# mynameisfiber/baton

Hardware: NVIDIA H100
Metric: federated local samples/sec (whole box), ResNet-18 FedAvg, synthetic non-IID 32x32 shards (higher is better)
Workload: dtype bf16

## Files before the change

### baton_b200/csrc/bindings.cpp

```cpp
#include <ATen/cuda/CUDAContext.h>
#include <c10/cuda/CUDAGuard.h>
#include <torch/extension.h>

#include <optional>
#include <vector>

#include "launch.h"

namespace {

inline cudaStream_t cur_stream() { return at::cuda::getCurrentCUDAStream().stream(); }
inline void check(int rc, const char* what) {
  TORCH_CHECK(rc == 0, "baton_b200::", what, " failed with code ", rc,
              rc > 0 ? std::string(" (") + cudaGetErrorString(static_cast<cudaError_t>(rc)) + ")" : std::string());
}
inline const void* cptr(const at::Tensor& t) { return t.data_ptr(); }
inline void* ptr(at::Tensor& t) { return t.data_ptr(); }
template <class T>
inline T* opt_ptr(const std::optional<at::Tensor>& t) {
  return (t.has_value() && t->defined()) ? reinterpret_cast<T*>(t->data_ptr()) : nullptr;
}
#define CHECK_CUDA(x) TORCH_CHECK((x).is_cuda(), #x " must be a CUDA tensor")

inline const float* prox_anchor(const std::optional<at::Tensor>& anchor, int64_t numel, const at::Tensor& hyper) {
// ... 289 lines not shown
  const int64_t nout = out.numel() / rows;
  TORCH_CHECK(w.numel() == (dgrad ? c * 9 * nout : nout * 9 * c), "conv_smallmap: w must be [Cout, 9*Cin]");
  TORCH_CHECK(dgrad ? !col_stats.has_value()
                    : (!col_stats.has_value() || (col_stats->scalar_type() == at::kFloat && col_stats->numel() >= 2 * nout)),
              "conv_smallmap: col_stats is a [2 Cout] fp32 buffer of the forward");
  const c10::cuda::CUDAGuard guard(src.device());
  const int rc = b200_conv_smallmap(cptr(src), cptr(w), ptr(out), static_cast<int>(src.size(0)),
                                    static_cast<int>(src.size(1)), static_cast<int>(src.size(2)), static_cast<int>(c),
                                    static_cast<int>(nout), static_cast<int>(stride), dgrad ? 1 : 0, static_cast<int>(mc),
                                    static_cast<int>(bn), opt_ptr<float>(col_stats), cur_stream());
  if (rc == -2) return false;
  check(rc, "conv_smallmap");
  return true;
}
bool conv_igemm_dgrad_s2(const at::Tensor& dy, const at::Tensor& w, at::Tensor dx, int64_t kh, int64_t kw,
                         const std::vector<int64_t>& ntaps, const std::vector<int64_t>& taps, int64_t force_bn) {
  CHECK_CUDA(dy); CHECK_CUDA(w); CHECK_CUDA(dx);
  TORCH_CHECK(dy.scalar_type() == at::kBFloat16 && w.scalar_type() == at::kBFloat16 && dx.scalar_type() == at::kBFloat16 &&
              dy.dim() == 4 && dx.dim() == 4 && dy.is_contiguous() && w.is_contiguous() && dx.is_contiguous());
  TORCH_CHECK(ntaps.size() == 4 && taps.size() == 16, "conv_igemm_dgrad_s2: 4 classes x 4 taps");
  int nt[4], tw[16];
  for (int i = 0; i < 4; ++i) nt[i] = static_cast<int>(ntaps[i]);
  for (int i = 0; i < 16; ++i) tw[i] = static_cast<int>(taps[i]);
  const c10::cuda::CUDAGuard guard(dy.device());
  const int rc = b200_conv_igemm_dgrad_s2(cptr(dy), cptr(w), ptr(dx), static_cast<int>(dx.size(0)),
                                          static_cast<int>(dx.size(1)), static_cast<int>(dx.size(2)),
                                          static_cast<int>(dx.size(3)), static_cast<int>(dy.size(3)), static_cast<int>(kh),
                                          static_cast<int>(kw), static_cast<int>(dy.size(1)), static_cast<int>(dy.size(2)),
                                          nt, tw, static_cast<int>(force_bn), cur_stream());
  if (rc == -2) return false;
  check(rc, "conv_igemm_dgrad_s2");
  return true;
}
bool conv_igemm_wgrad(const at::Tensor& dy, const at::Tensor& x, at::Tensor dw, int64_t cout, int64_t kh, int64_t kw,
                      int64_t stride, int64_t pad, int64_t ho, int64_t wo, int64_t split_k, int64_t force_bn,
                      const std::optional<at::Tensor>& sgd_theta, const std::optional<at::Tensor>& sgd_theta_bf16,
                      const std::optional<at::Tensor>& sgd_mom, const std::optional<at::Tensor>& sgd_hyper,
                      bool sgd_nesterov, const std::optional<at::Tensor>& sgd_anchor,
                      const std::optional<at::Tensor>& sgd_corr, const std::optional<at::Tensor>& sgd_v) {
  CHECK_CUDA(dy); CHECK_CUDA(x); CHECK_CUDA(dw);
  TORCH_CHECK(x.scalar_type() == at::kBFloat16 && dy.scalar_type() == at::kBFloat16 && dw.scalar_type() == at::kFloat &&
              x.dim() == 4 && x.is_contiguous() && dy.is_contiguous());
  const c10::cuda::CUDAGuard guard(x.device());
  const std::optional<B200SgdEpilogue> sgd =
      sgd_epilogue(sgd_theta, sgd_theta_bf16, sgd_mom, sgd_hyper, sgd_nesterov, sgd_anchor, sgd_corr, sgd_v);
  const int rc = b200_conv_igemm_wgrad(cptr(dy), cptr(x), dw.data_ptr<float>(), static_cast<int>(x.size(0)),
                                       static_cast<int>(x.size(1)), static_cast<int>(x.size(2)), static_cast<int>(x.size(3)),
                                       static_cast<int>(cout), static_cast<int>(kh), static_cast<int>(kw),
                                       static_cast<int>(stride), static_cast<int>(pad), static_cast<int>(ho),
                                       static_cast<int>(wo), static_cast<int>(split_k), static_cast<int>(force_bn),
                                       sgd ? &*sgd : nullptr, cur_stream());
  if (rc == -2 || rc == B200_SGD_EPILOGUE_DECLINED) return false;
  check(rc, "conv_igemm_wgrad");
  return true;
}

void gemm_fp8(const at::Tensor& a, const at::Tensor& b, at::Tensor d, const std::optional<at::Tensor>& bias,
              const std::optional<at::Tensor>& sfa, const std::optional<at::Tensor>& sfb, int64_t M, int64_t N, int64_t K,
              int64_t lda, int64_t ldb, int64_t ldd, int64_t act, int64_t split_k, bool accumulate, double alpha) {
  CHECK_CUDA(a); CHECK_CUDA(b); CHECK_CUDA(d);
  TORCH_CHECK(a.element_size() == 1 && b.element_size() == 1, "gemm_fp8 operands must be 1-byte (e4m3)");
  const c10::cuda::CUDAGuard guard(a.device());
  check(b200_gemm_fp8(cptr(a), cptr(b), ptr(d), opt_ptr<const float>(bias), opt_ptr<const void>(sfa),
                      opt_ptr<const void>(sfb), M, N, K, lda, ldb, ldd, d.scalar_type() == at::kFloat, act, split_k,
                      accumulate, static_cast<float>(alpha), cur_stream()),
        "gemm_fp8");
}
void quant_mx_rows(const at::Tensor& x, at::Tensor q, at::Tensor sf, int64_t R, int64_t C, int64_t ld_in, int64_t Cp) {
  CHECK_CUDA(x);
  const c10::cuda::CUDAGuard guard(x.device());
  check(b200_quant_mx_rows(x.data_ptr(), q.data_ptr(), sf.data_ptr(), R, C, ld_in, Cp, cur_stream()), "quant_mx_rows");
}
void quant_mx_cols(const at::Tensor& x, at::Tensor q, at::Tensor sf, int64_t R, int64_t C, int64_t ld_in, int64_t Rp) {
  CHECK_CUDA(x);
  const c10::cuda::CUDAGuard guard(x.device());
  check(b200_quant_mx_cols(x.data_ptr(), q.data_ptr(), sf.data_ptr(), R, C, ld_in, Rp, cur_stream()), "quant_mx_cols");
}

void fused_sgd(at::Tensor w, at::Tensor g, const std::optional<at::Tensor>& mom, const std::optional<at::Tensor>& wb,
               const at::Tensor& hyper, bool zero_grad, bool nesterov, const std::optional<at::Tensor>& wire_slot,
               const std::optional<at::Tensor>& pack_global, const std::optional<at::Tensor>& pack_scale, int64_t n_pack,
               bool wire_fp32, const std::optional<at::Tensor>& prox_anchor_, const std::optional<at::Tensor>& corr,
               const std::optional<at::Tensor>& adam_v, bool clip) {
  CHECK_CUDA(w);
  TORCH_CHECK(w.scalar_type() == at::kFloat && g.scalar_type() == at::kFloat && hyper.scalar_type() == at::kFloat);
  TORCH_CHECK(w.is_contiguous() && g.is_contiguous() && w.numel() == g.numel());
  const c10::cuda::CUDAGuard guard(w.device());
  const float* anchor = prox_anchor(prox_anchor_, w.numel(), hyper);
  const float* c = scaf_corr(corr, w.numel(), anchor);
  float* v = adam_v_ptr(adam_v, w.numel(), opt_ptr<float>(mom), hyper, anchor, c);
  check_clip_hyper(clip, hyper, v != nullptr);
  check(b200_fused_sgd(w.data_ptr<float>(), g.data_ptr<float>(), opt_ptr<float>(mom), opt_ptr<void>(wb), w.numel(),
                       hyper.data_ptr<float>(), zero_grad, nesterov,
                       reinterpret_cast<const unsigned long long*>(opt_ptr<const int64_t>(wire_slot)),
                       opt_ptr<const float>(pack_global), opt_ptr<const float>(pack_scale), n_pack, wire_fp32, anchor,
                       c, v, clip ? 1 : 0, cur_stream()),
        "fused_sgd");
}

void fused_sgd_segments(at::Tensor w, at::Tensor g, const std::optional<at::Tensor>& mom,
                        const std::optional<at::Tensor>& wb, const at::Tensor& segments, const at::Tensor& hyper,
                        bool nesterov, const std::optional<at::Tensor>& prox_anchor_,
                        const std::optional<at::Tensor>& corr, const std::optional<at::Tensor>& adam_v, bool clip) {
  CHECK_CUDA(w); CHECK_CUDA(segments);
  TORCH_CHECK(w.scalar_type() == at::kFloat && g.scalar_type() == at::kFloat && hyper.scalar_type() == at::kFloat);
  TORCH_CHECK(segments.scalar_type() == at::kLong && segments.dim() == 2 && segments.size(1) == 3 &&
// ... 1161 lines not shown
                            d.scalar_type() == at::kFloat, static_cast<int>(act), static_cast<float>(alpha), &l,
                            cur_stream()),
        "gemm_bf16_lora");
}

void lora_down(const at::Tensor& x, int64_t ldx, const at::Tensor& w, int64_t w_ts, int64_t wsj, int64_t wsk,
               at::Tensor u, int64_t ldu, int64_t M, int64_t T, int64_t rs, int64_t kt, const std::vector<int64_t>& xoff) {
  check_bf16(x, "lora_down x"); check_bf16(w, "lora_down w"); check_bf16(u, "lora_down u");
  TORCH_CHECK(static_cast<int64_t>(xoff.size()) == T, "lora_down: one x offset per slice");
  const c10::cuda::CUDAGuard guard(x.device());
  std::vector<long long> xo(xoff.begin(), xoff.end());
  check(b200_lora_down(cptr(x), ldx, cptr(w), w_ts, wsj, wsk, ptr(u), ldu, M, T, rs, kt, xo.data(), cur_stream()),
        "lora_down");
}

void lora_grad(const at::Tensor& l, int64_t ldl, const at::Tensor& q, int64_t ldq, at::Tensor out, int64_t osa,
               int64_t osb, int64_t out_ts, int64_t M, int64_t NA, int64_t NB, int64_t T, const std::vector<int64_t>& lo,
               const std::vector<int64_t>& qo, double s, at::Tensor work) {
  check_bf16(l, "lora_grad l"); check_bf16(q, "lora_grad q");
  CHECK_CUDA(out); CHECK_CUDA(work);
  TORCH_CHECK(out.scalar_type() == at::kFloat && work.scalar_type() == at::kFloat, "lora_grad: fp32 out and work");
  TORCH_CHECK(static_cast<int64_t>(lo.size()) == T && static_cast<int64_t>(qo.size()) == T, "lora_grad: offsets per slice");
  const int64_t splits = (M + B200_LORA_SPLIT_ROWS - 1) / B200_LORA_SPLIT_ROWS;
  TORCH_CHECK(work.numel() >= T * splits * NA * NB, "lora_grad: work holds T * splits * NA * NB floats");
  const c10::cuda::CUDAGuard guard(l.device());
  std::vector<long long> lo_(lo.begin(), lo.end()), qo_(qo.begin(), qo.end());
  check(b200_lora_grad(cptr(l), ldl, cptr(q), ldq, out.data_ptr<float>(), osa, osb, out_ts, M, NA, NB, T, lo_.data(),
                       qo_.data(), static_cast<float>(s), work.data_ptr<float>(), cur_stream()),
        "lora_grad");
}

}

PYBIND11_MODULE(TORCH_EXTENSION_NAME, m) {
  m.doc() = "baton_b200 sm_90a kernels";
  m.attr("MAX_RANKS") = B200_MAX_RANKS;
  m.def("gemm", &gemm);
  m.def("gemm_lora", &gemm_lora);
  m.def("lora_down", &lora_down);
  m.def("lora_grad", &lora_grad);
  m.attr("LORA_MAX_R") = B200_LORA_MAX_R;
  m.attr("LORA_SPLIT_ROWS") = B200_LORA_SPLIT_ROWS;
  m.def("trace_set", &trace_set);
  m.def("attention_fwd", &attention_fwd);
  m.def("attention_bwd", &attention_bwd);
  m.def("attention_short_fwd", &attention_short_fwd);
  m.def("attention_short_bwd", &attention_short_bwd);
  m.def("bn_bwd_cluster", &bn_bwd_cluster);
  m.def("gn_fwd", &gn_fwd);
  m.def("gn_bwd", &gn_bwd);
  m.def("im2col_tma_probe", &im2col_tma_probe);
  m.def("conv_igemm_fwd", &conv_igemm_fwd);
  m.def("conv_igemm_wgrad", &conv_igemm_wgrad);
  m.def("conv_igemm_dgrad", &conv_igemm_dgrad);
  m.def("conv_igemm_dgrad_s2", &conv_igemm_dgrad_s2);
  m.def("conv_halo", &conv_halo);
  m.def("conv_smallmap", &conv_smallmap);
  m.def("gemm_batched", &gemm_batched);
  m.def("gemm_fp8", &gemm_fp8);
  m.def("quant_mx_rows", &quant_mx_rows);
  m.def("quant_mx_cols", &quant_mx_cols);
  m.def("fused_sgd", &fused_sgd);
  m.def("fused_sgd_segments", &fused_sgd_segments);
  m.def("grad_norm_clip", &grad_norm_clip);
  m.attr("GRAD_NORM_WORK_WORDS") = B200_GRAD_NORM_WORK_WORDS;
  m.def("weighted_sum", &weighted_sum);
  m.def("fold_client", &fold_client);
  m.def("scaffold_corr", &scaffold_corr);
  m.def("scaffold_dc", &scaffold_dc);
  m.def("cast", &cast);
  m.def("gather_rows", &gather_rows);
  m.def("gather_augment", &gather_augment);
  m.def("gather_mix", &gather_mix);
  m.def("colsum", &colsum);
  m.def("add_bf16", &add_bf16);
  m.def("relu_bwd", &relu_bwd);
  m.def("gelu", &gelu);
  m.def("gelu_bwd", &gelu_bwd);
  m.def("gelu_erf", &gelu_erf);
  m.def("gelu_erf_bwd", &gelu_erf_bwd);
  m.def("vit_tokens_fwd", &vit_tokens_fwd);
  m.def("vit_tokens_bwd", &vit_tokens_bwd);
  m.def("pad_rows", &pad_rows);
  m.def("embedding_bwd", &embedding_bwd);
  m.def("fedavg_allreduce", &fedavg_allreduce);
  m.def("fedavg_allreduce_robust", &fedavg_allreduce_robust);
  m.def("fedavg_allreduce_krum", &fedavg_allreduce_krum);
  m.attr("KRUM_MAX_CTAS") = B200_KRUM_MAX_CTAS;
  m.attr("KRUM_PAIRS") = B200_KRUM_PAIRS;
  m.attr("KRUM_REPORT") = B200_KRUM_REPORT;
  m.def("fedavg_allreduce_topk", &fedavg_allreduce_topk);
  m.def("fedavg_allreduce_local", &fedavg_allreduce_local);
  m.def("fedavg_allreduce_secagg", &fedavg_allreduce_secagg);
  m.def("secagg_encode", &secagg_encode);
  m.def("topk_pack", &topk_pack);
  m.def("topk_fold", &topk_fold);
  m.def("nonzero_pack", &nonzero_pack);
  m.def("topk_work_words", [](int64_t n) { return static_cast<int64_t>(B200_TOPK_WORK_WORDS(n)); });
  m.def("pack_client", &pack_client);
  m.attr("MAX_ROBUST_CLIENTS") = B200_MAX_ROBUST_CLIENTS;
  m.attr("DP_WORK_WORDS") = B200_DP_WORK_WORDS;
  m.def("dp_clip_factor", &dp_clip_factor);
  m.def("fold_client_scaled", &fold_client_scaled);
  m.def("im2col", &im2col);
  m.def("col2im", &col2im);
  m.def("maxpool", &maxpool);
// ... 31 lines not shown
```

### baton_b200/csrc/gemm_wgmma.cu

```cuda
#define B200_TU_TAG 1
#include "ptx.cuh"
#include "epilogue.cuh"
#include "launch.h"
#include "pdl.cuh"
#include "sgd.cuh"

namespace b200 {

constexpr int BM = 128;
constexpr int BK = 64;
constexpr int WG_K = 16;
constexpr int GEMM_THREADS = 384;
constexpr int CONSUMER_WARPS = 8;
constexpr int CONSUMER_THREADS = 32 * CONSUMER_WARPS;
constexpr int MAX_STAGES = 8;
constexpr int S2_MAX_TAPS = 4;

struct GemmParams {
  int M, N, K;
  void* D;
  long long ldd;
  const float* bias;
  int out_fp32;
  int act;
// ... 1555 lines not shown
  p.ldb = static_cast<long long>(KH) * KW * Cin;
  p.flag_bias_off = -1; p.flag_epoch_ptr = nullptr;
  p.batched = 0; p.batch_inner = 1; p.batch_count = 1; p.d_outer = 0; p.d_inner = 0;
  p.conv_ho = Ho; p.conv_wo = Wo; p.conv_stride = 2; p.conv_pad = 0; p.conv_kw = KW; p.conv_cin = Cout;
  p.conv_taps = KH * KW; p.conv_ncol = Cin; p.conv_h = H; p.conv_w = W;
  dim3 grid((Cin + bn - 1) / bn, static_cast<unsigned>(4 * tiles_m), 1);
  if (bn == 128) return launch_fixed<128, 6, 4>(ta, tb, p, grid, stream);
  return launch_fixed<64, 8, 4>(ta, tb, p, grid, stream);
}

extern "C" int b200_conv_igemm_wgrad(const void* dy, const void* x, float* dw, int N, int H, int W, int Cin, int Cout,
                                     int KH, int KW, int stride, int pad, int Ho, int Wo, int split_k, int force_bn,
                                     const B200SgdEpilogue* sgd, cudaStream_t stream) {
  using namespace b200;
  const long long Mp = static_cast<long long>(N) * Ho * Wo;
  const int Kc = KH * KW * Cin;
  if (Mp <= 0 || Cout <= 0) return 0;
  if (Cin % 64 != 0 || Cout % 8 != 0 || Mp > (1ll << 30) || (reinterpret_cast<uintptr_t>(x) & 15) ||
      (reinterpret_cast<uintptr_t>(dy) & 15) || (reinterpret_cast<uintptr_t>(dw) & 15))
    return -2;
  const int bn = clamp_bn(force_bn > 0 ? force_bn : (Kc > 64 ? 128 : 64));
  CUtensorMap ta, tb;
  int rc = make_map(&ta, dy, Mp, Cout, Cout, 64, BK);
  if (rc) return rc;
  rc = b200_encode_map_im2col_bf16(&tb, x, N, H, W, Cin, KH, KW, stride, pad, 64, 64);
  if (rc) return rc;
  const int k_tiles = static_cast<int>((Mp + BK - 1) / BK);
  if (split_k < 1) split_k = 1;
  if (split_k > k_tiles) split_k = k_tiles;
  const int per = (k_tiles + split_k - 1) / split_k;
  split_k = (k_tiles + per - 1) / per;
  if (sgd != nullptr && split_k != 1) return B200_SGD_EPILOGUE_DECLINED;
  GemmParams p;
  if (sgd != nullptr) set_sgd_epilogue(p, *sgd);
  p.M = Cout; p.N = Kc; p.K = static_cast<int>(Mp); p.D = dw; p.ldd = Kc; p.bias = nullptr; p.out_fp32 = 1; p.act = 0;
  p.a_mn = 1; p.b_mn = 1; p.k_tiles_per_split = per; p.cluster_k = 1; p.atomic_out = 1;
  p.col_stats = nullptr;
  p.tile_flags = nullptr; p.flag_epoch = 0; p.alpha = 1.0f; p.flag_elem_off = 0; p.flag_tile_elems = 0; p.ldb = Kc;
  p.flag_bias_off = -1; p.flag_epoch_ptr = nullptr;
  p.batched = 0; p.batch_inner = 1; p.batch_count = 1; p.d_outer = 0; p.d_inner = 0;
  p.stages = 4;
  p.conv_ho = Ho; p.conv_wo = Wo; p.conv_stride = stride; p.conv_pad = pad; p.conv_kw = KW; p.conv_cin = Cin;
  p.conv_taps = KH * KW; p.conv_ncol = Cin;
  dim3 grid((Kc + bn - 1) / bn, (Cout + BM - 1) / BM, split_k);
  if (sgd != nullptr) {
    if (bn == 128) return launch_fixed_sgd<128, 6, 2>(ta, tb, p, grid, stream);
    return launch_fixed_sgd<64, 8, 2>(ta, tb, p, grid, stream);
  }
  if (bn == 128) return launch_fixed<128, 6, 2>(ta, tb, p, grid, stream);
  return launch_fixed<64, 8, 2>(ta, tb, p, grid, stream);
}

B200_TRACE_REGISTER(gemm_wgmma)
```

### baton_b200/csrc/launch.h

```cpp
#pragma once
#include <cuda_runtime.h>
#include <stdint.h>

#define B200_MAX_RANKS 16

extern "C" {

struct B200SgdEpilogue {
  float* theta;
  void* theta_bf16;
  float* mom;
  const float* hyper;
  int nesterov;
  const float* anchor;
  const float* corr;
  float* v;
};
#define B200_SGD_EPILOGUE_DECLINED (-6)

struct B200AffineEpilogue {
  const float* scale;
  const float* shift;
  const void* residual;
  long long ldr;
// ... 3 lines not shown

#define B200_LORA_MAX_R 192
struct B200LoraEpilogue {
  const void* u;
  long long ldu;
  const void* f;
  long long fs_n, fs_j;
  int R, rs, ds;
  int slot[3];
  float s;
};
int b200_gemm_bf16_lora(const void* a, const void* b, void* d, const float* bias, int M, int N, int K, long long lda,
                        long long ldb, long long ldd, int a_mn, int b_mn, int out_fp32, int act, float alpha,
                        const B200LoraEpilogue* lora, cudaStream_t stream);
int b200_lora_down(const void* x, long long ldx, const void* w, long long w_ts, long long wsj, long long wsk, void* u,
                   long long ldu, int M, int T, int rs, int kt, const long long* xoff, cudaStream_t stream);
#define B200_LORA_SPLIT_ROWS 256
int b200_lora_grad(const void* l, long long ldl, const void* q, long long ldq, float* out, long long osa, long long osb,
                   long long out_ts, int M, int NA, int NB, int T, const long long* lo, const long long* qo, float s,
                   float* work, cudaStream_t stream);

int b200_gemm_bf16(const void* a, const void* b, void* d, const float* bias, int M, int N, int K, long long lda,
                   long long ldb, long long ldd, int a_mn, int b_mn, int out_fp32, int act, int split_k, int accumulate,
                   float alpha, const uint32_t* tile_flags, uint32_t flag_epoch, long long flag_elem_off, int flag_tile_elems,
                   long long flag_bias_off, int force_bn, float* col_stats, const uint32_t* flag_epoch_ptr,
                   const B200SgdEpilogue* sgd, const B200AffineEpilogue* affine, cudaStream_t stream);
int b200_gemm_bf16_batched(const void* a, const void* b, void* d, int M, int N, int K, long long lda, long long ldb,
                           long long ldd, int a_mn, int b_mn, int out_fp32, int act, float alpha, int n_outer,
                           int n_inner, long long a_outer, long long a_inner, long long b_outer, long long b_inner,
                           long long d_outer, long long d_inner, int accumulate, cudaStream_t stream);
int b200_attention_fwd(const void* qkv, void* out, void* probs, int B, int S, int H, int dh, float scale,
                       cudaStream_t stream);
int b200_attention_bwd(const void* qkv, const void* dout, const void* probs, void* dqkv, int B, int S, int H, int dh,
                       float scale, cudaStream_t stream);
struct B200Dropout;
int b200_attention_drop_fwd(const void* qkv, void* out, void* probs, int B, int S, int H, int dh, float scale,
                            const B200Dropout* drop, cudaStream_t stream);
int b200_attention_drop_bwd(const void* qkv, const void* dout, const void* probs, void* dqkv, int B, int S, int H, int dh,
                            float scale, const B200Dropout* drop, cudaStream_t stream);
int b200_attention_short_fwd(const void* qkv, void* out, void* probs, int B, int S, int H, int dh, float scale,
                             cudaStream_t stream);
int b200_attention_short_bwd(const void* qkv, const void* dout, const void* probs, void* dqkv, int B, int S, int H, int dh,
                             float scale, cudaStream_t stream);
int b200_conv_igemm_fwd(const void* x, const void* w, void* y, int N, int H, int W, int Cin, int Cout, int KH, int KW,
                        int stride, int pad, int Ho, int Wo, int cluster_k, int force_bn, float* col_stats,
                        const B200AffineEpilogue* affine, cudaStream_t stream);
int b200_conv_igemm_dgrad(const void* dy, const void* w, void* dx, int N, int H, int W, int Cin, int Cout, int KH, int KW,
                          int pad, int Ho, int Wo, int cluster_k, int force_bn, cudaStream_t stream);
int b200_conv_igemm_dgrad_s2(const void* dy, const void* w, void* dx, int N, int H, int W, int Cin, int Cout, int KH,
                             int KW, int Ho, int Wo, const int* ntaps, const int* taps, int force_bn, cudaStream_t stream);
int b200_conv_igemm_wgrad(const void* dy, const void* x, float* dw, int N, int H, int W, int Cin, int Cout, int KH, int KW,
                          int stride, int pad, int Ho, int Wo, int split_k, int force_bn, const B200SgdEpilogue* sgd,
                          cudaStream_t stream);
int b200_conv_halo(const void* src, const void* w, void* out, int N, int H, int W, int C, int Nout, int stride,
                   int dgrad, int mc, float* col_stats, cudaStream_t stream);
int b200_conv_smallmap(const void* src, const void* w, void* out, int N, int H, int W, int C, int Nout, int stride,
                       int dgrad, int mc, int bn, float* col_stats, cudaStream_t stream);
int b200_im2col_tma_probe(const void* x, void* col, int N, int H, int W, int C, int KH, int KW, int stride, int pad,
                          int Ho, int Wo, cudaStream_t stream);
int b200_gemm_fp8(const void* a, const void* b, void* d, const float* bias, const void* sfa, const void* sfb, int M, int N,
                  int K, long long lda, long long ldb, long long ldd, int out_fp32, int act, int split_k, int accumulate,
                  float alpha, cudaStream_t stream);
int b200_quant_mx_rows(const void* x, void* q, void* sf, long long R, int C, long long ld_in, int Cp, cudaStream_t stream);
int b200_quant_mx_cols(const void* x, void* q, void* sf, long long R, int C, long long ld_in, long long Rp,
                       cudaStream_t stream);
int b200_gemm_simt(const void* a, const void* b, void* d, const float* bias, int M, int N, int K, long long lda,
                   long long ldb, long long ldd, int a_mn, int b_mn, int out_fp32, int act, int accumulate,
                   float alpha, cudaStream_t stream);

int b200_fused_sgd(float* w, float* g, float* mom, void* w_bf16, long long n, const float* hyper, int zero_grad,
                   int nesterov, const unsigned long long* wire_slot, const float* pack_global,
                   const float* pack_scale, long long n_pack, int wire_fp32, const float* prox_anchor,
                   const float* corr, float* adam_v, int clip, cudaStream_t stream);
int b200_fused_sgd_segments(float* w, float* g, float* mom, void* w_bf16, const long long* segments, int n_seg,
                            const float* hyper, int nesterov, const float* prox_anchor, const float* corr,
                            float* adam_v, int clip, cudaStream_t stream);
#define B200_GRAD_NORM_BLOCKS 528
#define B200_GRAD_NORM_WORK_WORDS (B200_GRAD_NORM_BLOCKS + 2)
int b200_grad_norm_clip(const float* g, long long n, const float* max_norm, void* work, float* norm_out,
                        float* coef_out, cudaStream_t stream);
int b200_scaffold_corr(float* corr, const float* c, const float* ci, long long n, cudaStream_t stream);
int b200_scaffold_dc(float* up, float* ci, const float* c, const float* global_w, const float* theta, long long n,
                     float inv_k_eta, int first, cudaStream_t stream);
int b200_fold_client(float* acc, float* theta, const float* global_w, void* w_bf16, float* mom, long long n_mom, long long n,
                     float nk, int mode, int reset, cudaStream_t stream);
int b200_weighted_sum(void* dst, const void* const* srcs, const float* weights, int n_src, long long n, int dtype,
                      cudaStream_t stream);
int b200_cast_f32_bf16(const float* src, void* dst, long long n, cudaStream_t stream);
int b200_cast_bf16_f32(const void* src, float* dst, long long n, cudaStream_t stream);
int b200_gather_rows(const void* src, const long long* idx, void* dst, long long n_rows, long long row_bytes,
                     cudaStream_t stream);
int b200_gather_rows_i64(const long long* src, const long long* idx, long long* dst, long long n,
                         cudaStream_t stream);
int b200_gather_augment(const void* src, const long long* idx, void* dst, const unsigned* words, long long n_rows,
                        long long s0, unsigned long long key, int pad, int crop, int flip, int H, int W, int C,
                        int elem_bytes, cudaStream_t stream);
int b200_gather_mix(const void* src, const long long* idx, void* dst, const unsigned* words, const int* rows,
                    long long n_rows, long long s0, int batch, unsigned long long key, int pad, int crop, int flip,
                    int H, int W, int C, int elem_bytes, int fp16, cudaStream_t stream);
int b200_colsum(const void* x, float* out, long long rows, int cols, int accumulate, cudaStream_t stream);
int b200_add_bf16(const void* a, const void* b, void* out, long long n, int relu, cudaStream_t stream);
int b200_relu_bwd_bf16(const void* y, const void* dy, void* dx, long long n, cudaStream_t stream);
int b200_gelu_bf16(const void* x, void* y, long long n, cudaStream_t stream);
int b200_gelu_bwd_bf16(const void* x, const void* dy, void* dx, long long n, cudaStream_t stream);
int b200_gelu_erf_bf16(const void* x, void* y, long long n, cudaStream_t stream);
int b200_gelu_erf_bwd_bf16(const void* x, const void* dy, void* dx, long long n, cudaStream_t stream);
// ... 218 lines not shown
```

### baton_b200/ops/functional.py

```python
from __future__ import annotations

import collections
import functools
from typing import List, Optional, Sequence, Tuple

import torch

from ._ext import load

BF16 = torch.bfloat16
NUM_SMS = 132


def _pitch(t: torch.Tensor) -> int:
    assert t.dim() == 2 and (t.stride(1) == 1 or t.shape[1] == 1), "GEMM operand must have unit inner stride"
    return t.stride(0) if t.shape[0] > 1 else max(t.stride(0), t.shape[1])


def _tma_ok(t: torch.Tensor) -> bool:
    return t.dtype == BF16 and _pitch(t) % 8 == 0 and t.data_ptr() % 16 == 0


def pick_bn(M: int, N: int) -> int:
    m_tiles = (M + 127) // 128
# ... 558 lines not shown
    return classes


def conv_igemm_dgrad(dy: torch.Tensor, w2d: torch.Tensor, in_shape, kh: int, kw: int, pad: int, stride: int = 1,
                     out: Optional[torch.Tensor] = None, path: Optional[str] = None,
                     mc: Optional[int] = None, cluster_k: Optional[int] = None) -> Optional[torch.Tensor]:
    n, h, w, c = in_shape
    cout = dy.shape[-1]
    if c % 64 or cout % 64 or w2d.shape[1] != kh * kw * c or not dy.is_contiguous() or not w2d.is_contiguous():
        return None
    kind = _conv_path(path, halo_eligible(kh, kw, stride, pad, cout, h, w, dgrad=True),
                      smallmap_eligible(kh, kw, stride, pad, cout, h, w, dgrad=True) and c % SMALLMAP_BN == 0)
    if kind == "halo":
        dx = out if out is not None else torch.empty((n, h, w, c), dtype=BF16, device=dy.device)
        if not load().conv_halo(dy, w2d, dx, 1, True, mc or halo_cluster(n * h * w), None):
            raise RuntimeError("conv_halo declined a convolution halo_eligible admits")
        return dx
    if kind == "smallmap":
        dx = out if out is not None else torch.empty((n, h, w, c), dtype=BF16, device=dy.device)
        if not load().conv_smallmap(dy, w2d, dx, 1, True, mc or halo_cluster(n * h * w), SMALLMAP_BN, None):
            raise RuntimeError("conv_smallmap declined a convolution smallmap_eligible admits")
        return dx
    if stride == 1:
        M, K = n * h * w, kh * kw * cout
        bn = pick_bn(M, c)
        dx = out if out is not None else torch.empty((n, h, w, c), dtype=BF16, device=dy.device)
        if cluster_k is None:
            cluster_k = pick_cluster_k(M, c, K, bn)
        ok = load().conv_igemm_dgrad(dy, w2d, dx, kh, kw, pad, cluster_k, bn)
        return dx if ok else None
    if stride != 2:
        return None
    ho, wo = dy.shape[1], dy.shape[2]
    classes = conv_s2_dgrad_taps(kh, kw, pad, ho, wo)
    if classes is None:
        return None
    bn = pick_bn(4 * n * ho * wo, c)
    words = [[t | dp << 16 | dq << 24 for t, dp, dq in taps] + [0] * (S2_MAX_TAPS - len(taps)) for taps in classes]
    dx = out if out is not None else torch.empty((n, h, w, c), dtype=BF16, device=dy.device)
    ok = load().conv_igemm_dgrad_s2(dy, w2d, dx, kh, kw, [len(t) for t in classes], [x for ws in words for x in ws], bn)
    return dx if ok else None


def conv_igemm_wgrad_(dy2d: torch.Tensor, x: torch.Tensor, dw2d: torch.Tensor, kh: int, kw: int, stride: int,
                      pad: int, sgd: Optional[dict] = None) -> bool:
    n, h, w, c = x.shape
    cout = dy2d.shape[1]
    if c % 64 or not x.is_contiguous() or not dy2d.is_contiguous() or not dw2d.is_contiguous():
        return False
    ho, wo = conv_out_size(h, kh, stride, pad), conv_out_size(w, kw, stride, pad)
    M, K = n * ho * wo, kh * kw * c
    bn = pick_bn(cout, K)
    split_k = pick_split_k(cout, K, M, bn)
    if sgd is not None and split_k != 1:
        return False
    sg = sgd or {}
    return bool(load().conv_igemm_wgrad(dy2d, x, dw2d, cout, kh, kw, stride, pad, ho, wo, split_k, bn,
                                        sg.get("theta"), sg.get("theta_bf16"), sg.get("momentum"), sg.get("hyper"),
                                        bool(sg.get("nesterov", False)), sg.get("anchor"), sg.get("corr"),
                                        sg.get("adam_v")))


def col2im(col: torch.Tensor, shape: Tuple[int, int, int, int], kh: int, kw: int, stride: int, pad: int,
           ho: int, wo: int) -> torch.Tensor:
    n, h, w, c = shape
    dx = torch.empty(shape, dtype=BF16, device=col.device)
    load().col2im(col, dx, n, h, w, c, kh, kw, stride, pad, ho, wo, col.shape[1])
    return dx


def maxpool(x: torch.Tensor, k: int, stride: int, pad: int) -> Tuple[torch.Tensor, torch.Tensor]:
    n, h, w, c = x.shape
    ho, wo = conv_out_size(h, k, stride, pad), conv_out_size(w, k, stride, pad)
    y = torch.empty((n, ho, wo, c), dtype=BF16, device=x.device)
    arg = torch.empty((n, ho, wo, c), dtype=torch.uint8 if (c % 8 == 0 and k * k <= 255) else torch.int32, device=x.device)
    load().maxpool(x, y, arg, n, h, w, c, k, stride, pad, ho, wo)
    return y, arg


def maxpool_bwd(dy: torch.Tensor, arg: torch.Tensor, in_shape, k: int, stride: int, pad: int,
                dy_b: Optional[torch.Tensor] = None) -> torch.Tensor:
    n, h, w, c = in_shape
    if dy_b is not None and arg.dtype != torch.uint8:
        dy, dy_b = add(dy, dy_b), None
    dx = torch.empty(in_shape, dtype=BF16, device=dy.device)
    load().maxpool_bwd(dy, dy_b, arg, dx, n, h, w, c, dy.shape[1], dy.shape[2], k, stride, pad)
    return dx


def bn_relu_maxpool(z: torch.Tensor, sums: torch.Tensor, gamma, beta, rmean, rvar, nbt, eps: float, momentum: float,
                    k: int, stride: int, pad: int):
    n, h, w, c = z.shape
    if c % 8 or k * k > 255:
        return None
    ho, wo = conv_out_size(h, k, stride, pad), conv_out_size(w, k, stride, pad)
    p = torch.empty((n, ho, wo, c), dtype=BF16, device=z.device)
    arg = torch.empty((n, ho, wo, c), dtype=torch.uint8, device=z.device)
    mean = torch.empty(c, dtype=torch.float32, device=z.device)
    rstd = torch.empty(c, dtype=torch.float32, device=z.device)
    if not load().bn_relu_maxpool(z, p, arg, sums, gamma, beta, rmean, rvar, mean, rstd, nbt, n, h, w, c, k, stride, pad,
                                  ho, wo, eps, momentum):
        return None
    return p, arg, mean, rstd


def bn_maxpool_bwd(z: torch.Tensor, p: torch.Tensor, arg: torch.Tensor, dy_a: torch.Tensor, dy_b: Optional[torch.Tensor],
                   gamma, mean: torch.Tensor, rstd: torch.Tensor, sums_b: torch.Tensor, dgamma, dbeta, k: int, stride: int,
                   pad: int) -> Optional[torch.Tensor]:
    n, h, w, c = z.shape
    dz = torch.empty_like(z)
    if not load().bn_maxpool_bwd(z, p, arg, dy_a, dy_b, dz, gamma, mean, rstd, sums_b, dgamma, dbeta, n, h, w, c, k, stride,
                                 pad, p.shape[1], p.shape[2]):
        return None
# ... 143 lines not shown
```

Baseline: 230,500.

## Add lean split-K conv weight-gradient kernel with in-kernel last-CTA reduction

Adds a dedicated 64x64-tile implicit-GEMM wgrad kernel (one producer warp with TMA im2col, one consumer warpgroup with wgmma) that splits the pixel reduction across CTAs. Partial sums are written to a workspace, and the last-arriving CTA per tile, chosen via an atomic counter, reduces them and applies the plain accumulate or fused SGD/Adam epilogue. Split-K wgrad cases with Cout divisible by 64 are routed to it. This lets the optimizer epilogue fuse even when split-K is needed and avoids a separate reduction pass. The cost is extra fp32 workspace traffic and a persistent per-stream workspace.

```diff
diff --git a/baton_b200/csrc/bindings.cpp b/baton_b200/csrc/bindings.cpp
--- a/baton_b200/csrc/bindings.cpp
+++ b/baton_b200/csrc/bindings.cpp
@@ -365,6 +365,34 @@
                                        sgd ? &*sgd : nullptr, cur_stream());
   if (rc == -2 || rc == B200_SGD_EPILOGUE_DECLINED) return false;
   check(rc, "conv_igemm_wgrad");
+  return true;
+}
+
+bool conv_wgrad_lean(const at::Tensor& dy, const at::Tensor& x, at::Tensor dw, int64_t kh, int64_t kw, int64_t stride,
+                     int64_t pad, int64_t ho, int64_t wo, int64_t splits, at::Tensor ws, at::Tensor counters,
+                     const std::optional<at::Tensor>& sgd_theta, const std::optional<at::Tensor>& sgd_theta_bf16,
+                     const std::optional<at::Tensor>& sgd_mom, const std::optional<at::Tensor>& sgd_hyper,
+                     bool sgd_nesterov, const std::optional<at::Tensor>& sgd_anchor,
+                     const std::optional<at::Tensor>& sgd_corr, const std::optional<at::Tensor>& sgd_v) {
+  CHECK_CUDA(dy); CHECK_CUDA(x); CHECK_CUDA(dw); CHECK_CUDA(ws); CHECK_CUDA(counters);
+  TORCH_CHECK(x.scalar_type() == at::kBFloat16 && dy.scalar_type() == at::kBFloat16 && dw.scalar_type() == at::kFloat &&
+              x.dim() == 4 && x.is_contiguous() && dy.dim() == 2 && dy.is_contiguous() && dw.dim() == 2 &&
+              dw.stride(1) == 1 && ws.scalar_type() == at::kFloat && counters.scalar_type() == at::kInt);
+  const int64_t cout = dy.size(1), kc = kh * kw * x.size(3);
+  TORCH_CHECK(dw.size(0) == cout && dw.size(1) == kc && dy.size(0) == x.size(0) * ho * wo);
+  const int64_t tiles = (kc + 63) / 64 * (cout / 64);
+  TORCH_CHECK(ws.numel() >= splits * tiles * 64 * 64 && counters.numel() >= tiles, "conv_wgrad_lean: workspace too small");
+  const c10::cuda::CUDAGuard guard(x.device());
+  const std::optional<B200SgdEpilogue> sgd =
+      sgd_epilogue(sgd_theta, sgd_theta_bf16, sgd_mom, sgd_hyper, sgd_nesterov, sgd_anchor, sgd_corr, sgd_v);
+  const int rc = b200_conv_wgrad_lean(
+      cptr(dy), cptr(x), dw.data_ptr<float>(), dw.stride(0), static_cast<int>(x.size(0)), static_cast<int>(x.size(1)),
+      static_cast<int>(x.size(2)), static_cast<int>(x.size(3)), static_cast<int>(cout), static_cast<int>(kh),
+      static_cast<int>(kw), static_cast<int>(stride), static_cast<int>(pad), static_cast<int>(ho), static_cast<int>(wo),
+      static_cast<int>(splits), ws.data_ptr<float>(), reinterpret_cast<unsigned*>(counters.data_ptr<int>()),
+      sgd ? &*sgd : nullptr, cur_stream());
+  if (rc == -2) return false;
+  check(rc, "conv_wgrad_lean");
   return true;
 }
 
@@ -1632,6 +1660,7 @@
   m.def("im2col_tma_probe", &im2col_tma_probe);
   m.def("conv_igemm_fwd", &conv_igemm_fwd);
   m.def("conv_igemm_wgrad", &conv_igemm_wgrad);
+  m.def("conv_wgrad_lean", &conv_wgrad_lean);
   m.def("conv_igemm_dgrad", &conv_igemm_dgrad);
   m.def("conv_igemm_dgrad_s2", &conv_igemm_dgrad_s2);
   m.def("conv_halo", &conv_halo);
diff --git a/baton_b200/csrc/gemm_wgmma.cu b/baton_b200/csrc/gemm_wgmma.cu
--- a/baton_b200/csrc/gemm_wgmma.cu
+++ b/baton_b200/csrc/gemm_wgmma.cu
@@ -1631,3 +1631,220 @@
 }
 
 B200_TRACE_REGISTER(gemm_wgmma)
+
+namespace b200 {
+constexpr int LEAN_THREADS = 160;
+constexpr int LEAN_STAGES = 4;
+constexpr int LEAN_RED_BATCH = 3;
+constexpr int LEAN_OP_BYTES = 64 * BK * 2;
+constexpr int LEAN_STAGE_BYTES = 2 * LEAN_OP_BYTES;
+constexpr int LEAN_PITCH = 64 + 4;
+constexpr int LEAN_SMEM = LEAN_STAGES * LEAN_STAGE_BYTES + 2 * LEAN_STAGES * 8 + 16 + 1024;
+static_assert(64 * LEAN_PITCH * 4 <= LEAN_STAGES * LEAN_STAGE_BYTES, "the drained ring must hold the fp32 tile");
+
+template <bool SGD, bool PROX, bool SCAF, bool ADAM>
+__global__ void __launch_bounds__(LEAN_THREADS, 1)
+conv_wgrad_lean_kernel(const __grid_constant__ CUtensorMap tmA, const __grid_constant__ CUtensorMap tmB,
+                       const GemmParams p, float4* __restrict__ ws, unsigned* __restrict__ counters) {
+  extern __shared__ __align__(1024) uint8_t smem_raw[];
+  uint8_t* smem = reinterpret_cast<uint8_t*>((reinterpret_cast<uintptr_t>(smem_raw) + 1023) & ~uintptr_t(1023));
+  uint64_t* full_bar = reinterpret_cast<uint64_t*>(smem + LEAN_STAGES * LEAN_STAGE_BYTES);
+  uint64_t* empty_bar = full_bar + LEAN_STAGES;
+  int* last = reinterpret_cast<int*>(empty_bar + LEAN_STAGES);
+
+  griddep_launch_dependents();
+  const int warp = threadIdx.x >> 5;
+  const int n0 = blockIdx.x * 64, m0 = blockIdx.y * 64;
+  const int splits = gridDim.z;
+  const int tile = blockIdx.y * gridDim.x + blockIdx.x;
+  const int k_tiles_total = (p.K + BK - 1) / BK;
+  const int kt_begin = blockIdx.z * p.k_tiles_per_split;
+  const int num_kt = min(kt_begin + p.k_tiles_per_split, k_tiles_total) - kt_begin;
+
+  if (warp == 4 && elect_one()) {
+    tma_prefetch_desc(&tmA);
+    tma_prefetch_desc(&tmB);
+    for (int s = 0; s < LEAN_STAGES; ++s) {
+      mbar_init(&full_bar[s], 1);
+      mbar_init(&empty_bar[s], 4);
+    }
+    fence_barrier_init();
+  }
+  __syncthreads();
+  griddep_wait();
+
+  if (warp == 4) {
+    if (elect_one()) {
+      const int tap = n0 / p.conv_cin, c = n0 - tap * p.conv_cin;
+      const int fr = tap / p.conv_kw, fs = tap - fr * p.conv_kw;
+      for (int i = 0; i < num_kt; ++i) {
+        const int s = i % LEAN_STAGES;
+        mbar_wait(&empty_bar[s], ((i / LEAN_STAGES) & 1) ^ 1);
+        uint8_t* sa = smem + s * LEAN_STAGE_BYTES;
+        uint8_t* sb = sa + LEAN_OP_BYTES;
+        const int k0 = (kt_begin + i) * BK;
+        mbar_expect_tx(&full_bar[s], LEAN_STAGE_BYTES);
+        tma_load_2d(sa, &tmA, &full_bar[s], m0, k0);
+        const int q0 = k0 % p.conv_wo, t0 = k0 / p.conv_wo;
+        tma_load_im2col_4d(sb, &tmB, &full_bar[s], c, q0 * p.conv_stride - p.conv_pad,
+                           (t0 % p.conv_ho) * p.conv_stride - p.conv_pad, t0 / p.conv_ho, fs, fr);
+      }
+    }
+    return;
+  }
+
+  float acc[32];
+#pragma unroll
+  for (int j = 0; j < 32; ++j) acc[j] = 0.f;
+  int prev = -1;
+  for (int i = 0; i < num_kt; ++i) {
+    const int s = i % LEAN_STAGES;
+    mbar_wait(&full_bar[s], (i / LEAN_STAGES) & 1);
+    const uint32_t sa = smem_u32(smem + s * LEAN_STAGE_BYTES);
+    const uint32_t sb = sa + LEAN_OP_BYTES;
+    wgmma_fence();
+#pragma unroll
+    for (int k = 0; k < BK / WG_K; ++k)
+      wgmma_bf16<64>(acc, gmma_desc_sw128(sa + k * 2048, 8192, 1024), gmma_desc_sw128(sb + k * 2048, 8192, 1024), 1u,
+                     1, 1);
+    wgmma_commit();
+    wgmma_wait<1>();
+    if (prev >= 0 && lane_id() == 0) mbar_arrive(&empty_bar[prev]);
+    prev = s;
+  }
+  wgmma_wait<0>();
+  wgmma_fence_operands(acc);
+
+  if (splits > 1) {
+    const size_t n_tiles = static_cast<size_t>(gridDim.x) * gridDim.y;
+    float4* slot = ws + (static_cast<size_t>(blockIdx.z) * n_tiles + tile) * (8 * 128) + threadIdx.x;
+#pragma unroll
+    for (int j = 0; j < 8; ++j) slot[j * 128] = make_float4(acc[4 * j], acc[4 * j + 1], acc[4 * j + 2], acc[4 * j + 3]);
+    __threadfence();
+    named_bar_sync(1, 128);
+    if (threadIdx.x == 0) *last = atomicAdd(counters + tile, 1u) == static_cast<unsigned>(splits - 1);
+    named_bar_sync(1, 128);
+    if (!*last) return;
+    __threadfence();
+    const float4* src = ws + static_cast<size_t>(tile) * (8 * 128) + threadIdx.x;
+    const size_t zstride = n_tiles * (8 * 128);
+#pragma unroll
+    for (int j = 0; j < 8; ++j) {
+      const float4 v = __ldcg(src + j * 128);
+      acc[4 * j] = v.x; acc[4 * j + 1] = v.y; acc[4 * j + 2] = v.z; acc[4 * j + 3] = v.w;
+    }
+    for (int z0 = 1; z0 < splits; z0 += LEAN_RED_BATCH) {
+      float4 v[LEAN_RED_BATCH][8];
+#pragma unroll
+      for (int b = 0; b < LEAN_RED_BATCH; ++b)
+#pragma unroll
+        for (int j = 0; j < 8; ++j)
+          v[b][j] = z0 + b < splits ? __ldcg(src + (z0 + b) * zstride + j * 128) : make_float4(0.f, 0.f, 0.f, 0.f);
+#pragma unroll
+      for (int b = 0; b < LEAN_RED_BATCH; ++b) {
+        if (z0 + b < splits) {
+#pragma unroll
+          for (int j = 0; j < 8; ++j) {
+            acc[4 * j] += v[b][j].x; acc[4 * j + 1] += v[b][j].y; acc[4 * j + 2] += v[b][j].z;
+            acc[4 * j + 3] += v[b][j].w;
+          }
+        }
+      }
+    }
+    if (threadIdx.x == 0) counters[tile] = 0;
+  }
+
+  float* part = reinterpret_cast<float*>(smem);
+  wg_store_acc<64>(acc, part, LEAN_PITCH, 0);
+  named_bar_sync(1, 128);
+  const int lrow = threadIdx.x >> 1, cc = (threadIdx.x & 1) * 32;
+  const int row = m0 + lrow, col0 = n0 + cc;
+  if (row >= p.M || col0 >= p.N) return;
+  uint32_t r[32];
+  acc_ld_row32(part + lrow * LEAN_PITCH + cc, r);
+  float v[32];
+#pragma unroll
+  for (int j = 0; j < 32; ++j) v[j] = __uint_as_float(r[j]);
+  const size_t e = static_cast<size_t>(row) * p.ldd + col0;
+  if constexpr (SGD) {
+    const bool vec = (p.ldd % 4 == 0) &&
+                     ((reinterpret_cast<uintptr_t>(p.sgd_theta) | reinterpret_cast<uintptr_t>(p.sgd_mom) |
+                       (PROX ? reinterpret_cast<uintptr_t>(p.sgd_anchor) : 0) |
+                       (SCAF ? reinterpret_cast<uintptr_t>(p.sgd_corr) : 0) |
+                       (ADAM ? reinterpret_cast<uintptr_t>(p.sgd_v) : 0)) & 15) == 0 &&
+                     (reinterpret_cast<uintptr_t>(p.sgd_wb) & 7) == 0;
+    if constexpr (ADAM) adamw_epilogue_chunk(p, e, col0, v, vec);
+    else sgd_epilogue_chunk<PROX, SCAF>(p, e, col0, v, vec);
+  } else {
+    float* d = reinterpret_cast<float*>(p.D) + e;
+    if (col0 + 32 <= p.N && p.ldd % 4 == 0 && (reinterpret_cast<uintptr_t>(p.D) & 15) == 0) {
+#pragma unroll
+      for (int j = 0; j < 32; j += 4) {
+        float4 o = *reinterpret_cast<float4*>(d + j);
+        o.x += v[j]; o.y += v[j + 1]; o.z += v[j + 2]; o.w += v[j + 3];
+        *reinterpret_cast<float4*>(d + j) = o;
+      }
+    } else {
+#pragma unroll
+      for (int j = 0; j < 32; ++j) if (col0 + j < p.N) d[j] += v[j];
+    }
+  }
+}
+
+template <bool SGD = false, bool PROX = false, bool SCAF = false, bool ADAM = false>
+static int launch_lean(const CUtensorMap& ta, const CUtensorMap& tb, const GemmParams& p, dim3 grid, float4* ws,
+                       unsigned* counters, cudaStream_t stream) {
+  static bool configured = false;
+  if (!configured) {
+    cudaError_t e = cudaFuncSetAttribute(conv_wgrad_lean_kernel<SGD, PROX, SCAF, ADAM>,
+                                         cudaFuncAttributeMaxDynamicSharedMemorySize, LEAN_SMEM);
+    if (e != cudaSuccess) return static_cast<int>(e);
+    configured = true;
+  }
+  cudaError_t le = launch_pdl(conv_wgrad_lean_kernel<SGD, PROX, SCAF, ADAM>, grid, LEAN_THREADS, LEAN_SMEM, stream, ta,
+                              tb, p, ws, counters);
+  if (le != cudaSuccess) return static_cast<int>(le);
+  return static_cast<int>(cudaGetLastError());
+}
+
+static int launch_lean_sgd(const CUtensorMap& ta, const CUtensorMap& tb, const GemmParams& p, dim3 grid, float4* ws,
+                           unsigned* counters, cudaStream_t stream) {
+  if (p.sgd_anchor != nullptr && p.sgd_corr != nullptr) return -2;
+  if (p.sgd_v != nullptr) {
+    if (p.sgd_anchor != nullptr || p.sgd_corr != nullptr || p.sgd_mom == nullptr) return -2;
+    return launch_lean<true, false, false, true>(ta, tb, p, grid, ws, counters, stream);
+  }
+  if (p.sgd_corr != nullptr) return launch_lean<true, false, true>(ta, tb, p, grid, ws, counters, stream);
+  return p.sgd_anchor != nullptr ? launch_lean<true, true>(ta, tb, p, grid, ws, counters, stream)
+                                 : launch_lean<true>(ta, tb, p, grid, ws, counters, stream);
+}
+}
+
+extern "C" int b200_conv_wgrad_lean(const void* dy, const void* x, float* dw, long long ldd, int N, int H, int W,
+                                    int Cin, int Cout, int KH, int KW, int stride, int pad, int Ho, int Wo, int splits,
+                                    float* ws, unsigned* counters, const B200SgdEpilogue* sgd, cudaStream_t stream) {
+  using namespace b200;
+  const long long Mp = static_cast<long long>(N) * Ho * Wo;
+  const int Kc = KH * KW * Cin;
+  if (Mp <= 0 || Cout <= 0) return 0;
+  if (Cout % 64 != 0 || Cin % 64 != 0 || Mp > (1ll << 30) || splits < 1 ||
+      ((reinterpret_cast<uintptr_t>(x) | reinterpret_cast<uintptr_t>(dy) | reinterpret_cast<uintptr_t>(ws)) & 15))
+    return -2;
+  CUtensorMap ta, tb;
+  int rc = make_map(&ta, dy, Mp, Cout, Cout, 64, BK);
+  if (rc) return rc;
+  rc = b200_encode_map_im2col_bf16(&tb, x, N, H, W, Cin, KH, KW, stride, pad, 64, 64);
+  if (rc) return rc;
+  const int k_tiles = static_cast<int>((Mp + BK - 1) / BK);
+  if (splits > k_tiles) splits = k_tiles;
+  const int per = (k_tiles + splits - 1) / splits;
+  splits = (k_tiles + per - 1) / per;
+  GemmParams p{};
+  if (sgd != nullptr) set_sgd_epilogue(p, *sgd);
+  p.M = Cout; p.N = Kc; p.K = static_cast<int>(Mp); p.D = dw; p.ldd = ldd; p.k_tiles_per_split = per;
+  p.conv_ho = Ho; p.conv_wo = Wo; p.conv_stride = stride; p.conv_pad = pad; p.conv_kw = KW; p.conv_cin = Cin;
+  dim3 grid((Kc + 63) / 64, Cout / 64, splits);
+  auto* w4 = reinterpret_cast<float4*>(ws);
+  return sgd != nullptr ? launch_lean_sgd(ta, tb, p, grid, w4, counters, stream)
+                        : launch_lean(ta, tb, p, grid, w4, counters, stream);
+}
diff --git a/baton_b200/csrc/launch.h b/baton_b200/csrc/launch.h
--- a/baton_b200/csrc/launch.h
+++ b/baton_b200/csrc/launch.h
@@ -79,6 +79,9 @@
 int b200_conv_igemm_wgrad(const void* dy, const void* x, float* dw, int N, int H, int W, int Cin, int Cout, int KH, int KW,
                           int stride, int pad, int Ho, int Wo, int split_k, int force_bn, const B200SgdEpilogue* sgd,
                           cudaStream_t stream);
+int b200_conv_wgrad_lean(const void* dy, const void* x, float* dw, long long ldd, int N, int H, int W, int Cin, int Cout,
+                         int KH, int KW, int stride, int pad, int Ho, int Wo, int splits, float* ws, unsigned* counters,
+                         const B200SgdEpilogue* sgd, cudaStream_t stream);
 int b200_conv_halo(const void* src, const void* w, void* out, int N, int H, int W, int C, int Nout, int stride,
                    int dgrad, int mc, float* col_stats, cudaStream_t stream);
 int b200_conv_smallmap(const void* src, const void* w, void* out, int N, int H, int W, int C, int Nout, int stride,
diff --git a/baton_b200/ops/functional.py b/baton_b200/ops/functional.py
--- a/baton_b200/ops/functional.py
+++ b/baton_b200/ops/functional.py
@@ -634,6 +634,8 @@
     M, K = n * ho * wo, kh * kw * c
     bn = pick_bn(cout, K)
     split_k = pick_split_k(cout, K, M, bn)
+    if split_k != 1 and cout % 64 == 0:
+        return wgrad_lean_(dy2d, x, dw2d, kh, kw, stride, pad, sgd=sgd)
     if sgd is not None and split_k != 1:
         return False
     sg = sgd or {}
@@ -641,6 +643,51 @@
                                         sg.get("theta"), sg.get("theta_bf16"), sg.get("momentum"), sg.get("hyper"),
                                         bool(sg.get("nesterov", False)), sg.get("anchor"), sg.get("corr"),
                                         sg.get("adam_v")))
+
+
+LEAN_TARGET_CTAS = 132
+LEAN_KT_RANGE = (8, 16)
+
+
+def wgrad_lean_plan(cout: int, kc: int, mp: int) -> Tuple[int, int, int]:
+    tiles = (kc + 63) // 64 * ((cout + 63) // 64)
+    k_tiles = (mp + 63) // 64
+    lo, hi = LEAN_KT_RANGE
+    splits = max(1, LEAN_TARGET_CTAS // tiles)
+    splits = min(splits, max(1, k_tiles // lo))
+    splits = max(splits, -(-k_tiles // hi))
+    per = -(-k_tiles // splits)
+    return -(-k_tiles // per), tiles, per
+
+
+_LEAN_WS = {}
+
+
+def _lean_workspace(dev: torch.device, floats: int, tiles: int):
+    key = (dev, torch.cuda.current_stream(dev).cuda_stream)
+    ws = _LEAN_WS.get(key)
+    if ws is None or ws[0].numel() < floats or ws[1].numel() < tiles:
+        ws = (torch.empty(max(floats, 1 << 20), dtype=torch.float32, device=dev),
+              torch.zeros(max(tiles, 1024), dtype=torch.int32, device=dev))
+        _LEAN_WS[key] = ws
+    return ws
+
+
+def wgrad_lean_(dy2d: torch.Tensor, x: torch.Tensor, dw2d: torch.Tensor, kh: int, kw: int, stride: int, pad: int,
+                sgd: Optional[dict] = None) -> bool:
+    cout, kc, mp = dy2d.shape[1], dw2d.shape[1], dy2d.shape[0]
+    n, h, w, _ = x.shape
+    ho, wo = conv_out_size(h, kh, stride, pad), conv_out_size(w, kw, stride, pad)
+    splits, tiles, _ = wgrad_lean_plan(cout, kc, mp)
+    ws, counters = _lean_workspace(dy2d.device, splits * tiles * 4096, tiles)
+    sg = sgd or {}
+    ok = bool(load().conv_wgrad_lean(dy2d, x, dw2d, kh, kw, stride, pad, ho, wo, splits, ws, counters,
+                                     sg.get("theta"), sg.get("theta_bf16"), sg.get("momentum"), sg.get("hyper"),
+                                     bool(sg.get("nesterov", False)), sg.get("anchor"), sg.get("corr"),
+                                     sg.get("adam_v")))
+    if not ok and sgd is None:
+        raise RuntimeError("conv_wgrad_lean declined a weight gradient of {} x {} over {} pixels".format(cout, kc, mp))
+    return ok
 
 
 def col2im(col: torch.Tensor, shape: Tuple[int, int, int, int], kh: int, kw: int, stride: int, pad: int,
```

Measured after the change: 230,300 (median of 6 runs). No clear change (-0.1%).
